# atsuki-ichikawa/KoeMorph

Measured on AMD Instinct MI355X. Metric: blendshape frames/sec (52-coef, 256-win, d_model=256), higher is better.
Workload: dtype f32; 1 GPU; C2: 256 windows/GPU x 136448 samples (8.5 s @16 kHz) -> 1024-pt STFT, hop 533, 80-bin log-mel (257 frames) -> dual-stream attention d_model=256, 8 heads, window 256 -> 52 coefficients + EMA; from audio resident in HBM (rotating batches); windows_per_gpu=256, samples_per_window=136448, parallelism=window-sharded x1, no collective

## Files before the change

koemorph_amd/csrc/km_context.h:

```cpp
#pragma once

#include <cstdint>
#include <map>
#include <string>
#include <vector>

#include "koemorph.h"
#include "km_devbuf.h"

namespace km {

constexpr int kNumMouth = 28;
constexpr int kNumExpr = 24;
extern const int kMouthIdx[kNumMouth];
extern const int kExprIdx[kNumExpr];

struct HostParam {
    std::vector<int64_t> shape;
    std::vector<float> data;
    bool loaded = false;
};

struct Packed {
    std::vector<float> host;
// ... 2 lines not shown

constexpr int kMelRpWaves = 8;
constexpr int kMelRpGroups = 4;
constexpr int kMelRpRow = 580;

struct MelPlan {
    km_mel_config cfg{};
    int n_freq = 0;
    std::vector<float> window;
    std::vector<float> twiddle;
    std::vector<int32_t> fb_start;
    std::vector<int32_t> fb_count;
    std::vector<int32_t> fb_offset;
    std::vector<float> fb_weight;
    std::vector<int32_t> fbg_gid;
    std::vector<int32_t> fbg_desc;
    std::vector<float> fbg_weight;
    int fbg_extent = 0;
    DevBuf<float> d_window, d_twiddle;
    DevBuf<int32_t> d_fb_start, d_fb_count, d_fb_offset;
    DevBuf<float> d_fb_weight;
    DevBuf<int32_t> d_fbg_gid, d_fbg_desc;
    DevBuf<float> d_fbg_weight;
    bool uploaded = false;
};

struct Options {
    int core_split = 0;
    int seq_per_window = 0;
    int seq_assemble = 0;
    int generic_staged = 0;
    int mel_two_frame = 0;
    int emotion_separate = 0;
    int no_ln_fusion = 0, no_db_fusion = 0, no_score_fusion = 0, no_out_fusion = 0, no_v_fusion = 0;
    int legacy_no_merge = 0;
    int no_core_merge = 0;
    int core128 = 0;
    int legacy_no_tail_fusion = 0;
    int legacy_no_enc_fusion = 0;
    int legacy_no_attn_fusion = 0;
    int kmm_no_fuse = 0;
    int train_no_split = 0;
    int train_split_min_k = 0;
    int train_alone_max = 0;
    int train_no_dy_split = 0;
    int train_ln_fuse_rows = 0;
    int train_no_ln_fuse = 0;
    int train_colsum_gemm = 0;
    int train_no_fe_pack = 0;
    int train_attn_regs = 0;
    int train_no_dma = 0;
    int train_op_per_launch = 0;
    int train_bm32_below = 0;
    int train_tail_groups = 0;
};
void options_from_env(Options& o);
int set_option(struct Context* c, const char* name, long long value);

struct PerDeviceOnce {
    unsigned long long seen[4] = {0, 0, 0, 0};
    bool first(int device) {
        if (device < 0 || device >= 256) return true;
        const unsigned long long bit = 1ull << (device & 63);
        if (seen[device >> 6] & bit) return false;
        seen[device >> 6] |= bit;
        return true;
// ... 299 lines not shown
```

koemorph_amd/csrc/km_device.h:

```cpp
#pragma once

#include <hip/hip_runtime.h>

#include "koemorph.h"

namespace km {

struct LogParams {
    int log_mode;
    float amin, top_db, db_add, db_scale, log_eps;
};

__device__ __forceinline__ float clamp_lo(float x, float lo) { return __builtin_amdgcn_fmed3f(x, lo, __builtin_inff()); }
__device__ __forceinline__ float db10(float s, float amin) {
    return 3.01029995663981195f * __builtin_amdgcn_logf(clamp_lo(s, amin));
}

__device__ __forceinline__ void log_window_consts(const LogParams& p, float ref, float& ref_db, float& floor_db) {
    ref_db = db10(ref, p.amin);
    floor_db = (db10(ref, p.amin) - ref_db) - p.top_db;
}

__device__ __forceinline__ float db_finish(const LogParams& p, float dbs, float ref_db, float floor_db) {
    float v = dbs - ref_db;
// ... 32 lines not shown
__device__ __forceinline__ float log_one_t(const LogParams& p, float s, float ref_db, float floor_db) {
    if (MODE == KM_LOG_LN_EPS) return 0.693147180559945309f * __builtin_amdgcn_logf(s + p.log_eps);
    float v = db10(s, p.amin) - ref_db;
    v = clamp_lo(v, floor_db);
    return (v + p.db_add) * p.db_scale;
}

__device__ __forceinline__ float log_one(const LogParams& p, float s, float ref_db, float floor_db) {
    return p.log_mode == KM_LOG_LN_EPS ? log_one_t<KM_LOG_LN_EPS>(p, s, ref_db, floor_db)
                                       : log_one_t<KM_LOG_DB_MAX>(p, s, ref_db, floor_db);
}

template <int MODE>
__device__ __forceinline__ float4 log_four_t(const LogParams& p, float4 v, float ref_db, float floor_db) {
    return make_float4(log_one_t<MODE>(p, v.x, ref_db, floor_db), log_one_t<MODE>(p, v.y, ref_db, floor_db),
                       log_one_t<MODE>(p, v.z, ref_db, floor_db), log_one_t<MODE>(p, v.w, ref_db, floor_db));
}

__device__ __forceinline__ float row16_sum(float v) {
    v += __int_as_float(__builtin_amdgcn_update_dpp(0, __float_as_int(v), 0xB1, 0xF, 0xF, true));
    v += __int_as_float(__builtin_amdgcn_update_dpp(0, __float_as_int(v), 0x4E, 0xF, 0xF, true));
    v += __int_as_float(__builtin_amdgcn_update_dpp(0, __float_as_int(v), 0x141, 0xF, 0xF, true));
    v += __int_as_float(__builtin_amdgcn_update_dpp(0, __float_as_int(v), 0x140, 0xF, 0xF, true));
    return v;
}

struct EmoArgs {
    const float* emo = nullptr;
    int ED = 0;
    const float *wee_t = nullptr , *bee = nullptr, *lg = nullptr, *lb = nullptr, *we2 = nullptr, *be2 = nullptr,
                *w2 = nullptr, *b2 = nullptr;
    float* zemo = nullptr;
    int d = 256, DH = 128;
};

__device__ __forceinline__ void emotion_window_d256(const EmoArgs& e, int64_t b, float* scratch) {
    constexpr int d = 256, DH = 128;
    float* emo_s = scratch;
    float* e1 = scratch + 256;
    float* part = scratch + 512;
    const int tid = threadIdx.x, lane = tid & 63;
    if (tid < 256) emo_s[tid] = tid < e.ED ? e.emo[b * e.ED + tid] : 0.f;
    __syncthreads();
    {
        const int n = tid & 255, h = __builtin_amdgcn_readfirstlane(tid >> 8);
#pragma unroll 1
        for (int q = 2 * h; q < 2 * h + 2; ++q) {
            const float* wp = e.wee_t + (size_t)64 * q * d + n;
            float w[64];
#pragma unroll
            for (int u = 0; u < 64; ++u) w[u] = wp[u * d];
            float acc = 0.f;
#pragma unroll
            for (int u = 0; u < 64; u += 4) {
                const float4 x = *reinterpret_cast<const float4*>(emo_s + 64 * q + u);
                acc = fmaf(x.x, w[u], acc);
                acc = fmaf(x.y, w[u + 1], acc);
                acc = fmaf(x.z, w[u + 2], acc);
                acc = fmaf(x.w, w[u + 3], acc);
            }
            part[q * d + n] = acc;
        }
    }
    __syncthreads();
    if (tid < 256) {
        float s = e.bee[tid];
#pragma unroll
        for (int q = 0; q < 4; ++q) s += part[q * d + tid];
        e1[tid] = s;
    }
    __syncthreads();
    if (tid < 64) {
        float x[4], s = 0.f;
#pragma unroll
        for (int i = 0; i < 4; ++i) { x[i] = e1[lane + 64 * i]; s += x[i]; }
#pragma unroll
        for (int o = 32; o > 0; o >>= 1) s += __shfl_xor(s, o);
        const float mean = s * (1.0f / d);
        float v = 0.f;
#pragma unroll
        for (int i = 0; i < 4; ++i) { const float t = x[i] - mean; v += t * t; }
#pragma unroll
        for (int o = 32; o > 0; o >>= 1) v += __shfl_xor(v, o);
        const float rstd = 1.0f / sqrtf(v * (1.0f / d) + 1e-5f);
#pragma unroll
        for (int i = 0; i < 4; ++i) {
            const int c = lane + 64 * i;
            e1[c] = (x[i] - mean) * rstd * e.lg[c] + e.lb[c];
        }
    }
    __syncthreads();
    {
        const int m = tid & 127, h = tid >> 7;
#pragma unroll 1
        for (int q = 2 * h; q < 2 * h + 2; ++q) {
            const float* wp = e.we2 + (size_t)32 * q * DH + m;
            float w[32];
#pragma unroll
            for (int u = 0; u < 32; ++u) w[u] = wp[u * DH];
            float acc = 0.f;
#pragma unroll
            for (int u = 0; u < 32; u += 4) {
                const float4 x = *reinterpret_cast<const float4*>(e1 + 32 * q + u);
                acc = fmaf(x.x, w[u], acc);
                acc = fmaf(x.y, w[u + 1], acc);
                acc = fmaf(x.z, w[u + 2], acc);
                acc = fmaf(x.w, w[u + 3], acc);
            }
            part[q * DH + m] = acc;
        }
    }
    __syncthreads();
    if (tid < 64) {
        float s = 0.f;
#pragma unroll
        for (int i = 0; i < 2; ++i) {
            const int mm = lane + 64 * i;
            float hsum = e.be2[mm];
#pragma unroll
            for (int q = 0; q < 8; ++q) hsum += part[q * DH + mm];
            s += fmaxf(hsum, 0.f) * e.w2[mm];
        }
#pragma unroll
        for (int o = 32; o > 0; o >>= 1) s += __shfl_xor(s, o);
        if (lane == 0) e.zemo[b] = s + e.b2[0];
    }
    __syncthreads();
}

struct EmoShape { int d = 0, DH = 0; };

__device__ __forceinline__ void emotion_layer_f4(const float* __restrict__ w, int K, int N, const float* x, float* part) {
    const int tid = threadIdx.x;
    const int tpr = N >> 2;
    const int G = 512 / tpr;
    const int c4 = tid & (tpr - 1), g = tid / tpr;
    const int kc = (K + G - 1) / G;
    const int k0 = g * kc, k1 = (k0 + kc) < K ? (k0 + kc) : K;
    float4 acc = make_float4(0.f, 0.f, 0.f, 0.f);
    const float* wp = w + 4 * c4;
    for (int k = k0; k < k1; k += 16) {
        float4 wv[16];
#pragma unroll
        for (int u = 0; u < 16; ++u) wv[u] = (k + u) < k1 ? *reinterpret_cast<const float4*>(wp + (size_t)(k + u) * N) : make_float4(0.f, 0.f, 0.f, 0.f);
#pragma unroll
        for (int u = 0; u < 16; ++u) {
            const float xv = (k + u) < k1 ? x[k + u] : 0.f;
            acc.x = fmaf(xv, wv[u].x, acc.x); acc.y = fmaf(xv, wv[u].y, acc.y);
            acc.z = fmaf(xv, wv[u].z, acc.z); acc.w = fmaf(xv, wv[u].w, acc.w);
        }
    }
    *reinterpret_cast<float4*>(part + g * N + 4 * c4) = acc;
}

__device__ __forceinline__ void emotion_window_generic(const EmoArgs& e, const EmoShape sh, int64_t b, float* scratch) {
    const int d = sh.d, DH = sh.DH;
    float* emo_s = scratch;
    float* e1 = scratch + 256;
    float* part = e1 + d;
    const int tid = threadIdx.x, lane = tid & 63;
    if (tid < 256) emo_s[tid] = tid < e.ED ? e.emo[b * e.ED + tid] : 0.f;
// ... 45 lines not shown
```

koemorph_amd/csrc/km_host.cpp:

```cpp
#include <cctype>
#include <cmath>
#include <cstdlib>
#include <cstdarg>
#include <cstdio>
#include <cstring>

#include "km_context.h"
#include "km_kmmf.h"

namespace km {

const int kMouthIdx[kNumMouth] = {14, 15, 16, 17, 18, 19, 20, 21, 22, 23, 24, 25, 26, 27,
                                  28, 29, 30, 31, 32, 33, 34, 35, 36, 37, 38, 39, 40, 51};
const int kExprIdx[kNumExpr] = {0, 1, 2, 3, 4, 5, 6, 7, 8, 9, 10, 11, 12, 13,
                                41, 42, 43, 44, 45, 46, 47, 48, 49, 50};

static thread_local char g_err[512] = "";

void set_error(const char* fmt, ...) {
    va_list ap;
    va_start(ap, fmt);
    vsnprintf(g_err, sizeof(g_err), fmt, ap);
    va_end(ap);
}
// ... 576 lines not shown
                            (int32_t)((uint32_t)(st4 / 4) | ((uint32_t)steps << 8) | ((uint32_t)(off / 4) << 16));
                        p->fbg_extent = std::max(p->fbg_extent, st4 + 4 * steps);
                    }
                }
            if (p->fbg_extent > kMelRpRow || p->fbg_weight.size() / 4 > 65535) { p->fbg_gid.clear(); p->fbg_desc.clear(); }
        }
        if (p->fbg_weight.empty()) p->fbg_weight.assign(4, 0.0f);
    }
    return p;
}

static bool same_cfg(const km_mel_config& a, const km_mel_config& b) { return std::memcmp(&a, &b, sizeof(a)) == 0; }

MelPlan* find_or_add_plan(Context* c, const km_mel_config& cfg) {
    for (MelPlan* p : c->mel_plans)
        if (same_cfg(p->cfg, cfg)) return p;
    MelPlan* p = build_mel_plan(cfg);
    c->mel_plans.push_back(p);
    return p;
}

}

using namespace km;

namespace km { const char* last_error(); }

namespace km {
namespace {
struct OptName { const char* name; int Options::*field; };
const OptName kOptNames[] = {
    {"core_split", &Options::core_split}, {"seq_per_window", &Options::seq_per_window}, {"seq_assemble", &Options::seq_assemble},
    {"generic_staged", &Options::generic_staged}, {"mel_two_frame", &Options::mel_two_frame},
    {"emotion_separate", &Options::emotion_separate}, {"no_ln_fusion", &Options::no_ln_fusion},
    {"no_db_fusion", &Options::no_db_fusion}, {"no_score_fusion", &Options::no_score_fusion},
    {"no_out_fusion", &Options::no_out_fusion}, {"no_v_fusion", &Options::no_v_fusion}, {"no_core_merge", &Options::no_core_merge}, {"core128", &Options::core128}, {"legacy_no_merge", &Options::legacy_no_merge}, {"kmm_no_fuse", &Options::kmm_no_fuse}, {"legacy_no_attn_fusion", &Options::legacy_no_attn_fusion}, {"legacy_no_enc_fusion", &Options::legacy_no_enc_fusion}, {"legacy_no_tail_fusion", &Options::legacy_no_tail_fusion},
    {"train_no_split", &Options::train_no_split}, {"train_tail_groups", &Options::train_tail_groups}, {"train_bm32_below", &Options::train_bm32_below}, {"train_op_per_launch", &Options::train_op_per_launch}, {"train_split_min_k", &Options::train_split_min_k}, {"train_no_dma", &Options::train_no_dma}, {"train_attn_regs", &Options::train_attn_regs}, {"train_no_fe_pack", &Options::train_no_fe_pack}, {"train_colsum_gemm", &Options::train_colsum_gemm}, {"train_no_ln_fuse", &Options::train_no_ln_fuse}, {"train_ln_fuse_rows", &Options::train_ln_fuse_rows}, {"train_no_dy_split", &Options::train_no_dy_split}, {"train_alone_max", &Options::train_alone_max},
};
}

void options_from_env(Options& o) {
    for (const OptName& n : kOptNames) {
        std::string env = "KM_";
        for (const char* p = n.name; *p; ++p) env += (char)std::toupper((unsigned char)*p);
        if (const char* v = std::getenv(env.c_str())) o.*(n.field) = *v ? std::atoi(v) : 1;
    }
    if (std::getenv("KM_GENERIC_NO_LN_FUSION")) o.no_ln_fusion = 1;
    if (std::getenv("KM_GENERIC_NO_DB_FUSION")) o.no_db_fusion = 1;
    if (std::getenv("KM_GENERIC_NO_SCORE_FUSION")) o.no_score_fusion = 1;
    if (std::getenv("KM_GENERIC_NO_OUT_FUSION")) o.no_out_fusion = 1;
    if (std::getenv("KM_GENERIC_NO_V_FUSION")) o.no_v_fusion = 1;
}

int set_option(Context* c, const char* name, long long value) {
    for (const OptName& n : kOptNames)
        if (std::strcmp(n.name, name) == 0) {
            c->opt.*(n.field) = (int)value;
            return KM_OK;
        }
    return fail(KM_ERR_INVALID_ARG, "km_set_option: unknown option '%s'", name);
}
}

extern "C" {

int km_abi_version(void) { return KM_ABI_VERSION; }
const char* km_last_error(void) { return km::last_error(); }
// ... 273 lines not shown
```

koemorph_amd/csrc/km_mel.hip:

```cpp
#include <hip/hip_runtime.h>

#include <cstdlib>

#include "km_context.h"
#include "km_device.h"

namespace km {


namespace mel {
constexpr int FPB = 16;
constexpr int WAVES = 4;
constexpr int FFT_BUF = 1152;
}

__device__ __forceinline__ float2 cadd(float2 a, float2 b) { return make_float2(a.x + b.x, a.y + b.y); }
__device__ __forceinline__ float2 csub(float2 a, float2 b) { return make_float2(a.x - b.x, a.y - b.y); }
__device__ __forceinline__ float2 cmul(float2 a, float2 b) {
    return make_float2(a.x * b.x - a.y * b.y, a.x * b.y + a.y * b.x);
}

template <int R>
__device__ __forceinline__ float2 twiddle_const(float2 d, int idx) {
    const int s = idx * (16 / R);
// ... 255 lines not shown
                const int st = fbs[m], cnt = fbc[m];
                const float* wt = fbw + fbo[m];
                const float* pr = pw + fl * NFS + st;
                float acc = 0.f;
                if (fvalid) {
#pragma unroll 4
                    for (int i = par; i < cnt; i += 2) acc = fmaf(pr[i], wt[i], acc);
                }
                acc += __shfl_xor(acc, 16);
                if (par == 0) outs[fl * a.n_mels + m] = acc;
                vmax = fmaxf(vmax, acc);
            }
        }
        __syncthreads();
        const int nf_here = (a.n_frames - f0) < FPB ? (a.n_frames - f0) : FPB;
        float* dst = a.melpow + ((int64_t)b * a.n_frames + f0) * a.n_mels;
        for (int i = tid; i < nf_here * a.n_mels; i += 256) dst[i] = outs[i];
    }
#pragma unroll
    for (int o = 32; o > 0; o >>= 1) vmax = fmaxf(vmax, __shfl_xor(vmax, o));
    if (lane == 0) redmax[wave] = vmax;
    __syncthreads();
    if (tid == 0) {
        const float mx = fmaxf(fmaxf(redmax[0], redmax[1]), fmaxf(redmax[2], redmax[3]));
        atomicMax(a.melmax + b, __float_as_uint(mx));
    }
}

#ifndef KM_MEL_SKIP
#define KM_MEL_SKIP 0
#endif
#ifdef KM_MEL_STAMP
#define KM_ASM asm volatile
__device__ unsigned long long km_mel_stamps[1024 * 8 * 24];
#define KM_STAMP(i)                                                  \
    do {                                                             \
        const unsigned long long now_ = __builtin_readcyclecounter(); \
        st_acc[i] += (unsigned)(now_ - st_last);                     \
        st_last = now_;                                              \
    } while (0)
#else
#define KM_ASM asm
#define KM_STAMP(i) do {} while (0)
#endif
namespace melrp {
constexpr int WAVES = kMelRpWaves, NT = 64 * WAVES, FPB = 16, NC = 512, FFT_BUF = 576, NGW = kMelRpGroups;
constexpr int NFS = kMelRpRow;
static_assert(WAVES == 8 && NFS % 64 == 4 && NFS >= 528, "mel stage layout");

typedef float v2f __attribute__((ext_vector_type(2)));

#define KM_ADD(D, A, B) "v_pk_add_f32 %[" #D "], %[" #A "], %[" #B "]\n\t"
#define KM_SUB(D, A, B) "v_pk_add_f32 %[" #D "], %[" #A "], %[" #B "] neg_lo:[0,1] neg_hi:[0,1]\n\t"
#define KM_ADD_NI(D, A, B) "v_pk_add_f32 %[" #D "], %[" #A "], %[" #B "] op_sel:[0,1] op_sel_hi:[1,0] neg_hi:[0,1]\n\t"
#define KM_SUB_NI(D, A, B) "v_pk_add_f32 %[" #D "], %[" #A "], %[" #B "] op_sel:[0,1] op_sel_hi:[1,0] neg_lo:[0,1]\n\t"
#define KM_ROT3(D, S) "v_pk_add_f32 %[" #D "], %[" #S "], %[" #S "] op_sel:[1,0] op_sel_hi:[0,1] neg_lo:[0,1] neg_hi:[1,1]\n\t"
#define KM_CMUL1(T, A, W) "v_pk_mul_f32 %[" #T "], %[" #A "], %[" #W "] op_sel_hi:[0,1]\n\t"
#define KM_CMUL2(D, A, W, T) \
    "v_pk_fma_f32 %[" #D "], %[" #A "], %[" #W "], %[" #T "] op_sel:[1,1,0] op_sel_hi:[1,0,1] neg_lo:[1,0,0]\n\t"

__device__ __forceinline__ void dif8(v2f (&v)[8]) {
    constexpr float C2 = 0.70710678118654752f;
    const v2f c = {C2, C2};
    v2f r0 = v[0], r1 = v[1], r2 = v[2], r3 = v[3], r4 = v[4], r5 = v[5], r6 = v[6], r7 = v[7], t;
    KM_ASM("s_nop 0\n\t"
        KM_ADD(t, r0, r4) KM_SUB(r4, r0, r4)
        KM_ADD(r0, r1, r5) KM_SUB(r5, r1, r5)
// ... 68 lines not shown
                 "ds_read_b64 %5, %8 offset:%14\n\t"
                 "ds_read_b64 %6, %8 offset:%15\n\t"
                 "ds_read_b64 %7, %8 offset:%16\n\t"
                 "s_waitcnt lgkmcnt(0)"
                 : "=&v"(y[0]), "=&v"(y[1]), "=&v"(y[2]), "=&v"(y[3]), "=&v"(y[4]), "=&v"(y[5]), "=&v"(y[6]), "=&v"(y[7])
                 : "v"(addr), "i"(0 * S), "i"(1 * S), "i"(2 * S), "i"(3 * S), "i"(4 * S), "i"(5 * S), "i"(6 * S), "i"(7 * S)
                 : "memory");
}
template <int S>
__device__ __forceinline__ void lds_write8_bitrev(unsigned addr, const v2f (&y)[8]) {
    asm volatile("ds_write_b64 %8, %0 offset:%9\n\t"
                 "ds_write_b64 %8, %1 offset:%10\n\t"
                 "ds_write_b64 %8, %2 offset:%11\n\t"
                 "ds_write_b64 %8, %3 offset:%12\n\t"
                 "ds_write_b64 %8, %4 offset:%13\n\t"
                 "ds_write_b64 %8, %5 offset:%14\n\t"
                 "ds_write_b64 %8, %6 offset:%15\n\t"
                 "ds_write_b64 %8, %7 offset:%16"
                 :
                 : "v"(y[0]), "v"(y[1]), "v"(y[2]), "v"(y[3]), "v"(y[4]), "v"(y[5]), "v"(y[6]), "v"(y[7]), "v"(addr),
                   "i"(0 * S), "i"(4 * S), "i"(2 * S), "i"(6 * S), "i"(1 * S), "i"(5 * S), "i"(3 * S), "i"(7 * S)
                 : "memory");
}
__device__ __forceinline__ v2f ld2(const float2* p) { const float2 t = *p; return v2f{t.x, t.y}; }

#ifndef KM_MEL_XCHG
#define KM_MEL_XCHG 1
#endif
#ifndef KM_MEL_REMAP
#define KM_MEL_REMAP 1
#endif
#ifndef KM_MEL_FLAT
#define KM_MEL_FLAT 0
#endif
#ifndef KM_MEL_PRIO
#define KM_MEL_PRIO 3
#endif
#ifndef KM_MEL_W2
#define KM_MEL_W2 0
#endif
__device__ __forceinline__ void swap_lane32(v2f& a, v2f& b) {
    const auto r0 = __builtin_amdgcn_permlane32_swap(__float_as_uint(a.x), __float_as_uint(b.x), false, false);
    const auto r1 = __builtin_amdgcn_permlane32_swap(__float_as_uint(a.y), __float_as_uint(b.y), false, false);
    a = v2f{__uint_as_float(r0[0]), __uint_as_float(r1[0])}; b = v2f{__uint_as_float(r0[1]), __uint_as_float(r1[1])};
}
__device__ __forceinline__ void swap_lane16(v2f& a, v2f& b) {
    const auto r0 = __builtin_amdgcn_permlane16_swap(__float_as_uint(a.x), __float_as_uint(b.x), false, false);
    const auto r1 = __builtin_amdgcn_permlane16_swap(__float_as_uint(a.y), __float_as_uint(b.y), false, false);
    a = v2f{__uint_as_float(r0[0]), __uint_as_float(r1[0])}; b = v2f{__uint_as_float(r0[1]), __uint_as_float(r1[1])};
}
#define KM_XM " row_mask:0xf bank_mask:"
#define KM_XBANK(CT, MT, CA, MA, MB)                                      \
    "s_nop 1\n\t"                                                        \
    "v_mov_b32_dpp %[t0], %[a0] " CT KM_XM MT "\n\t"                      \
    "v_mov_b32_dpp %[t1], %[a1] " CT KM_XM MT "\n\t"                      \
    "v_mov_b32_dpp %[t2], %[a2] " CT KM_XM MT "\n\t"                      \
    "v_mov_b32_dpp %[t3], %[a3] " CT KM_XM MT "\n\t"                      \
    "v_mov_b32_dpp %[a0], %[b0] " CA KM_XM MA "\n\t"                      \
    "v_mov_b32_dpp %[a1], %[b1] " CA KM_XM MA "\n\t"                      \
    "v_mov_b32_dpp %[a2], %[b2] " CA KM_XM MA "\n\t"                      \
    "v_mov_b32_dpp %[a3], %[b3] " CA KM_XM MA "\n\t"                      \
    "v_mov_b32_dpp %[b0], %[t0] quad_perm:[0,1,2,3]" KM_XM MB "\n\t"      \
    "v_mov_b32_dpp %[b1], %[t1] quad_perm:[0,1,2,3]" KM_XM MB "\n\t"      \
    "v_mov_b32_dpp %[b2], %[t2] quad_perm:[0,1,2,3]" KM_XM MB "\n\t"      \
    "v_mov_b32_dpp %[b3], %[t3] quad_perm:[0,1,2,3]" KM_XM MB "\n\t"      \
    "s_nop 0"
// ... 164 lines not shown
    const int bx = TAB ? (b == 0 ? (int)blockIdx.x : 0) : (int)(lin_ / gridDim.y);
#else
    const int b = blockIdx.y, bx = (int)blockIdx.x;
    static_assert(!TAB, "the clip-span launch is laid out for KM_MEL_REMAP");
#endif
    const unsigned gx = TAB ? (b == 0 ? (unsigned)a.tab_span_wgs : 1u) : gridDim.x;
    const int n_frames = TAB && b > 0 ? 2 : a.n_frames;
    const int64_t gw = a.win0 + b;
    const int64_t clip = TAB ? 0 : gw / a.wins_per_clip;
    int tab_f0 = 0;
    if constexpr (TAB) { tab_f0 = b == 0 ? a.tab_min : a.tab_start[b - 1]; tab_f0 = tab_f0 < 0 ? 0 : tab_f0; }
    const int64_t woff = TAB ? (int64_t)tab_f0 * a.hop : (gw - clip * a.wins_per_clip) * a.win_step;
    const int64_t Lw = TAB ? (int64_t)(b == 0 ? a.n_frames - 1 : a.tab_T) * a.hop : a.L;
    const float* x = a.audio + clip * a.clip_len + (TAB && woff >= a.clip_len ? 0 : woff);
    const int Lv = (int)((a.clip_len - woff) < Lw ? (a.clip_len - woff) : Lw);
    if (a.ready && !a.ready[b]) return;
    const int rs = RING ? a.ring_start[b] : -1;
    v2f* buf = reinterpret_cast<v2f*>(fbuf + wave * FFT_BUF);
    const int n_chunks = (n_frames + FPB - 1) / FPB;
    const unsigned rd2 = lds_offset(buf + (lane >> 3) * 72 + (lane & 7)), rd3 = lds_offset(buf + lane * 9);
    const unsigned wr3 = lds_offset(buf + fft_lane_k0(lane) * 9 + (lane & 7));
    const int cbin = fft_lane_bin(lane);

    v2f zn[8];
    bool zn_ok = false;
    const int fmul = TAB ? (b == 0 ? 1 : a.tab_T) : a.frame_mul;
    auto first_frame = [&]() {
        if (KM_MEL_SKIP & 8) {
#pragma unroll
            for (int i = 0; i < 8; ++i) zn[i] = v2f{0.001f * lane, 0.5f + i};
            zn_ok = true;
        } else if (bx * FPB + wave < n_frames) zn_ok = load_frame_rp_fast<RING>(x, Lv, rs, a.hop, (bx * FPB + wave) * fmul, lane, zn);
    };
    if (!PACK && !TAB && !(KM_MEL_SKIP & 16) && a.emo.emo && bx == (int)gx - 1) {
        if (a.emo.d == 256 && a.emo.DH == 128) emotion_window_d256(a.emo, gw, pw);
        else emotion_window_generic(a.emo, EmoShape{a.emo.d, a.emo.DH}, gw, pw);
        first_frame();
    } else {
        first_frame();
    }

    const unsigned ctr_last = (unsigned)n_chunks - 1u;
    for (int i = tid; i < a.fbg_nw; i += NT) fbw[i] = a.fbg_weight[i];
    for (int i = tid; i < FPB * (NFS - 513); i += NT) pw[(i / (NFS - 513)) * NFS + 513 + i % (NFS - 513)] = 0.f;

    const int n2 = lane & 7, k0 = fft_lane_k0(lane);
    v2f win2[8], tw1[8], tw2[8], twp[4];
#pragma unroll
    for (int i = 0; i < 8; ++i) {
        win2[i] = v2f{a.window[2 * (lane + 64 * i)], a.window[2 * (lane + 64 * i) + 1]};
        tw1[i] = ld2(a.twiddle + ((2 * lane * bitrev(i, 3)) & 1023));
        tw2[i] = ld2(a.twiddle + ((16 * n2 * bitrev(i, 3)) & 1023));
    }
#pragma unroll
    for (int i = 0; i < 4; ++i) twp[i] = ld2(a.twiddle + cbin + 64 * i);

    int my_gid[NGW];
#pragma unroll
    for (int i = 0; i < NGW; ++i) my_gid[i] = __builtin_amdgcn_readfirstlane(a.fbg_gid[wave * NGW + i]);
    const int* my_desc_p = a.fbg_desc + wave * NGW * 4 + mel_slot_of_lane(lane);
#pragma unroll
    for (int i = 0; i < 8; ++i) asm volatile("" ::"v"(win2[i]), "v"(tw1[i]), "v"(tw2[i]));
#pragma unroll
    for (int i = 0; i < 4; ++i) asm volatile("" ::"v"(twp[i]));
#pragma unroll
    for (int i = 0; i < NGW; ++i) asm volatile("" ::"s"(my_gid[i]));

    float vmax = 0.f;
// ... 184 lines not shown
                    acc = __builtin_elementwise_fma(v2f{pv.z, pv.w}, v2f{wv.z, wv.w}, acc);
                    pv = pn; wv = wn;
                }
                acc = __builtin_elementwise_fma(v2f{pv.x, pv.y}, v2f{wv.x, wv.y}, acc);
                acc = __builtin_elementwise_fma(v2f{pv.z, pv.w}, v2f{wv.z, wv.w}, acc);
                float r = acc.x + acc.y;
                r = fvalid ? r : 0.f;
                asm("v_max_f32 %0, %0, %1" : "+v"(vmax) : "v"(r));
                asm("v_max_f32 %0, %0, %1" : "+v"(fmx) : "v"(r));
                store_mel(my_gid[i], r);
            }
#endif
            if (!TAB && a.frame_max) {
                float fall = fmx;
#pragma unroll
                for (int s2 = 0; s2 < 4; ++s2) fall = fmaxf(fall, __shfl(fmx, mel_lane_of(s2, flm)));
                fmx = fall;
                if (slot == 0 && fvalid) atomicMax(a.frame_max + (int64_t)b * n_frames + f0 + flm, __float_as_uint(fmx));
            }
        }
        if (KM_MEL_PRIO) __builtin_amdgcn_s_setprio(0);
        KM_STAMP(10);
        chunk = chunk_next;
        chunk_next = __builtin_amdgcn_readfirstlane(sched[0]);
        __syncthreads();
        KM_STAMP(11);
#ifdef KM_MEL_STAMP
        if (f0 + FPB > n_frames) st_acc[14] += (unsigned)(st_last - st_turn);
        else { st_acc[15] += (unsigned)(st_last - st_turn); }
#endif
    }
#ifdef KM_MEL_STAMP
    if (lane == 0) {
        unsigned long long* o = km_mel_stamps + ((size_t)(b * gridDim.x + bx) * WAVES + wave) * 24;
        if (b * gridDim.x + bx < 1024) {
            for (int i = 0; i < 12; ++i) o[i] = st_acc[i];
            o[12] = st_last - st_first;
            o[13] = st_entry; o[14] = st_first; o[15] = st_last; o[16] = st_entry_rt; o[17] = __builtin_amdgcn_s_memrealtime();
            o[18] = __builtin_readcyclecounter();
            o[19] = st_acc[12]; o[20] = st_acc[13]; o[21] = st_acc[14]; o[22] = st_acc[15];
        }
    }
#endif
#pragma unroll
    for (int o = 32; o > 0; o >>= 1) vmax = fmaxf(vmax, __shfl_xor(vmax, o));
    if (lane == 0) redmax[wave] = vmax;
    __syncthreads();
    if (!TAB && tid == 0 && !a.frame_max) {
        float mx = redmax[0];
#pragma unroll
        for (int w = 1; w < WAVES; ++w) mx = fmaxf(mx, redmax[w]);
        atomicMax(a.melmax + b, __float_as_uint(mx));
    }
}

struct LogArgs {
    const float* melpow;
    const unsigned* melmax;
    int n_frames, out_frames, n_mels;
    LogParams lp;
    float* mel_long;
    float* mel_short;
};

__global__ __launch_bounds__(256) void mel_log_kernel(LogArgs a) {
    const int b = blockIdx.y;
    float ref_db, floor_db;
    log_window_consts(a.lp, __uint_as_float(a.melmax[b]), ref_db, floor_db);
    const float* src = a.melpow + (int64_t)b * a.n_frames * a.n_mels;
    const int total = a.out_frames * a.n_mels;
    const int i = blockIdx.x * 256 + threadIdx.x;
    if (i < total) {
        int f = i / a.n_mels;
// ... 63 lines not shown
                    3 * n_mels + nnz) * sizeof(float);
}

static LogParams log_params(const km_mel_config& m) {
    LogParams lp;
    lp.log_mode = m.log_mode; lp.amin = m.amin; lp.top_db = m.top_db; lp.db_add = m.db_add;
    lp.db_scale = m.db_scale; lp.log_eps = m.log_eps;
    return lp;
}

int growth_refused(void* stream, const char* what, int64_t need, int64_t cap) {
    hipStreamCaptureStatus cs = hipStreamCaptureStatusNone;
    if (hipStreamIsCapturing((hipStream_t)stream, &cs) == hipSuccess && cs != hipStreamCaptureStatusNone)
        return fail(KM_ERR_WORKSPACE, "%s: %lld exceeds the %lld allocated during a stream capture: run one call with this span first",
                    what, (long long)need, (long long)cap);
    return KM_OK;
}

int ensure_chunk_counters(Context* c, int64_t windows, void* stream) {
    if (windows <= c->ws_chunkctr.n) return KM_OK;
    const int64_t cap_n = windows < 4096 ? 4096 : windows;
    if (int rc = c->ws_chunkctr.grow(cap_n, stream, "front end: windows of one launch")) return rc;
    HIP_TRY(hipMemsetAsync(c->ws_chunkctr, 0, (size_t)cap_n * sizeof(unsigned), (hipStream_t)stream));
    HIP_TRY(hipStreamSynchronize((hipStream_t)stream));
    return KM_OK;
}

bool mel_rp_ok(Context* c, MelPlan* p) { return p->cfg.n_fft == 1024 && !c->opt.mel_two_frame && p->d_fbg_gid != nullptr; }

bool clip_frames_shared(Context* c, MelPlan* p) {
    const km_mel_config& m = p->cfg;
    return m.pad_mode == KM_PAD_CONSTANT && 2 * m.hop_length >= m.n_fft && m.n_mels == c->NK && c->NK % 4 == 0;
}

bool mel_fuses_emotion(Context* c, MelPlan* p) {
    auto pow2 = [](int v) { return v >= 64 && v <= 1024 && (v & (v - 1)) == 0; };
    static const bool generic_ok = std::getenv("KM_EMOTION_GENERIC_SEPARATE") == nullptr;
    const bool d256 = c->d == 256 && c->DH == 128;
    return mel_rp_ok(c, p) && !c->opt.emotion_separate && c->kind == 0 && c->ED <= 256 && (d256 || (generic_ok && pow2(c->d) && pow2(c->DH)));
}

bool mel_packs(Context* c, MelPlan* p, int64_t n_frames, int64_t T) {
    const km_mel_config& m = p->cfg;
    return mel_rp_ok(c, p) && m.log_mode == KM_LOG_DB_MAX && m.top_db == m.db_add && m.db_scale > 0.f && n_frames >= T && n_frames >= 3;
}

static void mel_plan_args(MelPlan* p, MelArgs& a) {
    const km_mel_config& m = p->cfg;
    a.hop = m.hop_length; a.pad_mode = m.pad_mode;
    a.n_mels = m.n_mels; a.window = p->d_window; a.twiddle = reinterpret_cast<const float2*>(p->d_twiddle.p);
    a.fb_start = p->d_fb_start; a.fb_count = p->d_fb_count; a.fb_offset = p->d_fb_offset; a.fb_weight = p->d_fb_weight;
    a.fb_nnz = (int)p->fb_weight.size();
    a.fbg_gid = p->d_fbg_gid; a.fbg_desc = p->d_fbg_desc; a.fbg_weight = p->d_fbg_weight; a.fbg_nw = (int)p->fbg_weight.size();
}

int launch_mel_power(Context* c, MelPlan* p, const MelSrc& src, void* stream, const MelCarry& carry) {
    const km_mel_config& m = p->cfg;
    const SeqFrames* seq = carry.seq;
    const int64_t B = src.B, L = src.L;
    const int64_t n_frames = seq ? seq->n_rows : 1 + L / m.hop_length;
    if (m.pad_mode == KM_PAD_REFLECT && L <= m.n_fft / 2)
        return fail(KM_ERR_INVALID_ARG, "reflect padding needs more than n_fft/2 = %d samples (got %lld)", m.n_fft / 2, (long long)L);
    if (!seq && (B > c->ws.windows || n_frames > c->ws.frames))
        return fail(KM_ERR_WORKSPACE, "workspace holds %lld windows x %lld frames, need %lld x %lld: call km_reserve",
                    (long long)c->ws.windows, (long long)c->ws.frames, (long long)B, (long long)n_frames);
    if (!seq && m.n_mels > c->ws.mels)
// ... 6 lines not shown
    if (!p->uploaded) return fail(KM_ERR_NOT_FINALIZED, "mel plan not uploaded (km_finalize / km_reserve first)");
    static PerDeviceOnce once;
    if (once.first(c->device)) {
        const struct { const void* fn; int lds; } kernels[] = {
            {(const void*)&mel_power_kernel<1024, false>, (int)mel_lds_bytes(1024)}, {(const void*)&mel_power_kernel<512, false>, (int)mel_lds_bytes(512)},
            {(const void*)&mel_power_kernel<1024, true>, (int)mel_lds_bytes(1024)}, {(const void*)&mel_power_kernel<512, true>, (int)mel_lds_bytes(512)},
            {(const void*)&mel_power_rp_kernel<false>, 160 * 1024}, {(const void*)&mel_power_rp_kernel<true>, 160 * 1024},
            {(const void*)&mel_power_rp_kernel<false, true>, 160 * 1024}};
        for (const auto& k : kernels) HIP_TRY(hipFuncSetAttribute(k.fn, hipFuncAttributeMaxDynamicSharedMemorySize, k.lds));
    }
    hipStream_t st = (hipStream_t)stream;
    if (int rc = ensure_chunk_counters(c, B, stream)) return rc;
    if (!seq && c->melmax_dirty) {
        HIP_TRY(hipMemsetAsync(c->ws.melmax, 0, (size_t)c->ws.windows * sizeof(unsigned), st));
        c->melmax_dirty = false;
    }
    MelArgs a;
    mel_plan_args(p, a);
    a.audio = src.audio; a.L = L; a.clip_len = src.clip_len; a.win_step = src.win_step; a.win0 = src.win0;
    a.wins_per_clip = src.wins_per_clip > 0 ? src.wins_per_clip : 1; a.n_frames = (int)n_frames;
    a.ring_start = src.ring_start; a.ready = src.ready;
    a.melpow = c->ws.melpow; a.melmax = c->ws.melmax;
    a.frame_mul = 1; a.frame_max = nullptr; a.chunk_ctr = c->ws_chunkctr;
    a.pack_xt = nullptr; a.pack_T = a.pack_KP = 0; a.pack_amin = m.amin;
    a.tab_start = nullptr; a.tab_edge = nullptr; a.tab_min = a.tab_T = a.tab_span_wgs = 0;
    if (carry.pack) { a.pack_xt = carry.pack->xt; a.pack_T = carry.pack->T; a.pack_KP = carry.pack->KP; }
    if (seq) { a.melpow = seq->pow; a.frame_max = seq->fmax; a.frame_mul = seq->frame_mul; a.melmax = nullptr; }
    if (carry.emotion) {
        auto dvp = [&](const char* name) { return (const float*)c->packed.at(name).dev; };
        a.emo.emo = carry.emotion; a.emo.ED = c->ED; a.emo.zemo = carry.zemo;
        a.emo.d = c->d; a.emo.DH = c->DH;
        a.emo.wee_t = (c->d == 256 && c->DH == 128) ? dvp("wee_t256") : dvp("wee_t"); a.emo.bee = dvp("bee"); a.emo.lg = dvp("eln_g"); a.emo.lb = dvp("eln_b");
        a.emo.we2 = dvp("we2"); a.emo.be2 = dvp("be2"); a.emo.w2 = dvp("w2"); a.emo.b2 = dvp("b2");
    }
    const int n_chunks = (int)((n_frames + mel::FPB - 1) / mel::FPB);
    int per_window = (int)((512 + B / 2) / B);
    if (per_window > n_chunks) per_window = n_chunks;
    if (per_window < 1) per_window = 1;
    const dim3 grid((unsigned)per_window, (unsigned)B);
    if (mel_rp_ok(c, p)) {
        const size_t ldsrp = melrp_lds_bytes(a.fbg_nw);
        if (carry.pack) hipLaunchKernelGGL((mel_power_rp_kernel<false, true>), grid, dim3(melrp::NT), ldsrp, st, a);
        else if (!ring) hipLaunchKernelGGL((mel_power_rp_kernel<false>), grid, dim3(melrp::NT), ldsrp, st, a);
        else hipLaunchKernelGGL((mel_power_rp_kernel<true>), grid, dim3(melrp::NT), ldsrp, st, a);
        HIP_TRY(hipGetLastError());
        return KM_OK;
    }
    const size_t lds = mel_lds_bytes(m.n_fft, m.n_mels, a.fb_nnz);
    if (m.n_fft == 1024 && !ring) hipLaunchKernelGGL((mel_power_kernel<1024, false>), grid, dim3(256), lds, st, a);
    else if (m.n_fft == 1024) hipLaunchKernelGGL((mel_power_kernel<1024, true>), grid, dim3(256), lds, st, a);
    else if (!ring) hipLaunchKernelGGL((mel_power_kernel<512, false>), grid, dim3(256), lds, st, a);
    else hipLaunchKernelGGL((mel_power_kernel<512, true>), grid, dim3(256), lds, st, a);
    HIP_TRY(hipGetLastError());
    return KM_OK;
}

struct ClipPackArgs {
    const float* span;
    int edge_off;
    const int* start;
    int min_start, n_span, T, KP, n_mels, row_stride, tile_cols;
    float amin;
    float* xt;
    unsigned* melmax;
};
namespace clippack {
// ... 151 lines not shown
                                 unsigned char* __restrict__ ready, const float* __restrict__ samples,
                                 int n_in, int hop, int ring_len) {
    const int s = blockIdx.x;
    const int w0 = wptr[s];
    float* r = ring + (int64_t)s * ring_len;
    const float* in = samples + (int64_t)s * n_in;
    for (int i = threadIdx.x; i < hop; i += blockDim.x) {
        int p = w0 + i;
        p -= p >= ring_len ? ring_len : 0;
        r[p] = i < n_in ? in[i] : 0.f;
    }
    __syncthreads();
    if (threadIdx.x == 0) {
        int w = w0 + hop;
        w -= w >= ring_len ? ring_len : 0;
        wptr[s] = w;
        const int f = frames[s] + 1;
        frames[s] = f;
        if ((int64_t)f * hop >= ring_len) ready[s] = 1;
    }
}

int launch_ring_push(Context* c, const float* samples, int64_t n_per_stream, void* stream) {
    hipLaunchKernelGGL(ring_push_kernel, dim3((unsigned)c->st.n_streams), dim3(256), 0, (hipStream_t)stream, c->st.ring,
                       c->st.ring_wptr, c->st.ring_frames, c->st.ring_ready, samples, (int)n_per_stream, c->st.ring_hop,
                       (int)c->st.ring_len);
    HIP_TRY(hipGetLastError());
    return KM_OK;
}

LogParams plan_log_params(MelPlan* p) { return log_params(p->cfg); }

#ifdef KM_MEL_STAMP
extern "C" __attribute__((visibility("default"))) int km_debug_mel_stamps(unsigned long long* out, int n) {
    return (int)hipMemcpyFromSymbol(out, HIP_SYMBOL(km_mel_stamps), (size_t)n * sizeof(unsigned long long));
}
#endif

}
```

Baseline: 1.926 million frames/s.

## Batch emotion MLP across groups of windows in a single rider block

The emotion MLP, which rides on the last mel block of each window, now processes 2 (default) or 4 windows per rider block. Each weight column loaded into registers is reused across several windows' inputs. One window per group becomes the rider and the others skip emotion work. This cuts weight traffic and the number of blocks doing the extra work, but makes the rider blocks longer, which could worsen load imbalance. Debug cycle-stamp slots are also added under a compile flag.

```diff
diff --git a/koemorph_amd/csrc/km_context.h b/koemorph_amd/csrc/km_context.h
--- a/koemorph_amd/csrc/km_context.h
+++ b/koemorph_amd/csrc/km_context.h
@@ -58,6 +58,7 @@
     int generic_staged = 0;
     int mel_two_frame = 0;
     int emotion_separate = 0;
+    int emo_group = 0;
     int no_ln_fusion = 0, no_db_fusion = 0, no_score_fusion = 0, no_out_fusion = 0, no_v_fusion = 0;
     int legacy_no_merge = 0;
     int no_core_merge = 0;
diff --git a/koemorph_amd/csrc/km_device.h b/koemorph_amd/csrc/km_device.h
--- a/koemorph_amd/csrc/km_device.h
+++ b/koemorph_amd/csrc/km_device.h
@@ -88,16 +88,20 @@
                 *w2 = nullptr, *b2 = nullptr;
     float* zemo = nullptr;
     int d = 256, DH = 128;
+    int group = 1;
 };
 
-__device__ __forceinline__ void emotion_window_d256(const EmoArgs& e, int64_t b, float* scratch) {
+#define KM_EMO_STAMP(i) do { if (st) st[i] = __builtin_readcyclecounter(); } while (0)
+__device__ __forceinline__ void emotion_window_d256(const EmoArgs& e, int64_t b, float* scratch, unsigned long long* st = nullptr) {
     constexpr int d = 256, DH = 128;
     float* emo_s = scratch;
     float* e1 = scratch + 256;
     float* part = scratch + 512;
     const int tid = threadIdx.x, lane = tid & 63;
+    KM_EMO_STAMP(0);
     if (tid < 256) emo_s[tid] = tid < e.ED ? e.emo[b * e.ED + tid] : 0.f;
     __syncthreads();
+    KM_EMO_STAMP(1);
     {
         const int n = tid & 255, h = __builtin_amdgcn_readfirstlane(tid >> 8);
 #pragma unroll 1
@@ -118,6 +122,7 @@
             part[q * d + n] = acc;
         }
     }
+    KM_EMO_STAMP(2);
     __syncthreads();
     if (tid < 256) {
         float s = e.bee[tid];
@@ -146,6 +151,7 @@
         }
     }
     __syncthreads();
+    KM_EMO_STAMP(3);
     {
         const int m = tid & 127, h = tid >> 7;
 #pragma unroll 1
@@ -166,6 +172,7 @@
             part[q * DH + m] = acc;
         }
     }
+    KM_EMO_STAMP(4);
     __syncthreads();
     if (tid < 64) {
         float s = 0.f;
@@ -182,7 +189,135 @@
         if (lane == 0) e.zemo[b] = s + e.b2[0];
     }
     __syncthreads();
-}
+    KM_EMO_STAMP(5);
+}
+
+constexpr int kEmoGroupMax = 4;
+__host__ __device__ constexpr int emotion_group_floats(int nb) { return nb * (256 + 256) + 4 * nb * 256; }
+
+template <int NB>
+__device__ __forceinline__ void emotion_group_d256_n(const EmoArgs& e, int64_t b0, int nb, float* scratch, unsigned long long* st) {
+    constexpr int d = 256, DH = 128;
+    float* emo_s = scratch;
+    float* e1 = scratch + NB * 256;
+    float* part = scratch + NB * 512;
+    const int tid = threadIdx.x, lane = tid & 63, wave = tid >> 6;
+    KM_EMO_STAMP(0);
+    for (int i = tid; i < NB * 256; i += 512) {
+        const int w = i >> 8, k = i & 255;
+        emo_s[i] = (w < nb && k < e.ED) ? e.emo[(b0 + w) * e.ED + k] : 0.f;
+    }
+    __syncthreads();
+    KM_EMO_STAMP(1);
+    {
+        const int n = tid & 255, h = __builtin_amdgcn_readfirstlane(tid >> 8);
+#pragma unroll 1
+        for (int q = 2 * h; q < 2 * h + 2; ++q) {
+            const float* wp = e.wee_t + (size_t)64 * q * d + n;
+            float w[64];
+#pragma unroll
+            for (int u = 0; u < 64; ++u) w[u] = wp[u * d];
+            float acc[NB];
+#pragma unroll
+            for (int v = 0; v < NB; ++v) acc[v] = 0.f;
+#pragma unroll
+            for (int u = 0; u < 64; u += 4)
+#pragma unroll
+                for (int v = 0; v < NB; ++v) {
+                    const float4 x = *reinterpret_cast<const float4*>(emo_s + v * 256 + 64 * q + u);
+                    acc[v] = fmaf(x.x, w[u], acc[v]);
+                    acc[v] = fmaf(x.y, w[u + 1], acc[v]);
+                    acc[v] = fmaf(x.z, w[u + 2], acc[v]);
+                    acc[v] = fmaf(x.w, w[u + 3], acc[v]);
+                    if (v == NB - 1 && u % 16 == 12) __builtin_amdgcn_sched_barrier(0);
+                }
+#pragma unroll
+            for (int v = 0; v < NB; ++v) part[(q * NB + v) * d + n] = acc[v];
+        }
+    }
+    KM_EMO_STAMP(2);
+    __syncthreads();
+    for (int i = tid; i < NB * d; i += 512) {
+        const int v = i >> 8, n = i & 255;
+        float s = e.bee[n];
+#pragma unroll
+        for (int q = 0; q < 4; ++q) s += part[(q * NB + v) * d + n];
+        e1[i] = s;
+    }
+    __syncthreads();
+    if (wave < nb) {
+        float* ew = e1 + wave * d;
+        float x[4], s = 0.f;
+#pragma unroll
+        for (int i = 0; i < 4; ++i) { x[i] = ew[lane + 64 * i]; s += x[i]; }
+#pragma unroll
+        for (int o = 32; o > 0; o >>= 1) s += __shfl_xor(s, o);
+        const float mean = s * (1.0f / d);
+        float v = 0.f;
+#pragma unroll
+        for (int i = 0; i < 4; ++i) { const float t = x[i] - mean; v += t * t; }
+#pragma unroll
+        for (int o = 32; o > 0; o >>= 1) v += __shfl_xor(v, o);
+        const float rstd = 1.0f / sqrtf(v * (1.0f / d) + 1e-5f);
+#pragma unroll
+        for (int i = 0; i < 4; ++i) {
+            const int c = lane + 64 * i;
+            ew[c] = (x[i] - mean) * rstd * e.lg[c] + e.lb[c];
+        }
+    }
+    __syncthreads();
+    KM_EMO_STAMP(3);
+    {
+        const int m = tid & 127, h = tid >> 7;
+#pragma unroll 1
+        for (int q = 2 * h; q < 2 * h + 2; ++q) {
+            const float* wp = e.we2 + (size_t)32 * q * DH + m;
+            float w[32];
+#pragma unroll
+            for (int u = 0; u < 32; ++u) w[u] = wp[u * DH];
+            float acc[NB];
+#pragma unroll
+            for (int v = 0; v < NB; ++v) acc[v] = 0.f;
+#pragma unroll
+            for (int u = 0; u < 32; u += 4)
+#pragma unroll
+                for (int v = 0; v < NB; ++v) {
+                    const float4 x = *reinterpret_cast<const float4*>(e1 + v * d + 32 * q + u);
+                    acc[v] = fmaf(x.x, w[u], acc[v]);
+                    acc[v] = fmaf(x.y, w[u + 1], acc[v]);
+                    acc[v] = fmaf(x.z, w[u + 2], acc[v]);
+                    acc[v] = fmaf(x.w, w[u + 3], acc[v]);
+                    if (v == NB - 1 && u % 16 == 12) __builtin_amdgcn_sched_barrier(0);
+                }
+#pragma unroll
+            for (int v = 0; v < NB; ++v) part[(q * NB + v) * DH + m] = acc[v];
+        }
+    }
+    KM_EMO_STAMP(4);
+    __syncthreads();
+    if (wave < nb) {
+        float s = 0.f;
+#pragma unroll
+        for (int i = 0; i < 2; ++i) {
+            const int mm = lane + 64 * i;
+            float hsum = e.be2[mm];
+#pragma unroll
+            for (int q = 0; q < 8; ++q) hsum += part[(q * NB + wave) * DH + mm];
+            s += fmaxf(hsum, 0.f) * e.w2[mm];
+        }
+#pragma unroll
+        for (int o = 32; o > 0; o >>= 1) s += __shfl_xor(s, o);
+        if (lane == 0) e.zemo[b0 + wave] = s + e.b2[0];
+    }
+    __syncthreads();
+    KM_EMO_STAMP(5);
+}
+
+__device__ __forceinline__ void emotion_group_d256(const EmoArgs& e, int64_t b0, int nb, float* scratch, unsigned long long* st = nullptr) {
+    if (nb <= 2) emotion_group_d256_n<2>(e, b0, nb, scratch, st);
+    else emotion_group_d256_n<kEmoGroupMax>(e, b0, nb, scratch, st);
+}
+#undef KM_EMO_STAMP
 
 struct EmoShape { int d = 0, DH = 0; };
 
diff --git a/koemorph_amd/csrc/km_host.cpp b/koemorph_amd/csrc/km_host.cpp
--- a/koemorph_amd/csrc/km_host.cpp
+++ b/koemorph_amd/csrc/km_host.cpp
@@ -632,7 +632,7 @@
 const OptName kOptNames[] = {
     {"core_split", &Options::core_split}, {"seq_per_window", &Options::seq_per_window}, {"seq_assemble", &Options::seq_assemble},
     {"generic_staged", &Options::generic_staged}, {"mel_two_frame", &Options::mel_two_frame},
-    {"emotion_separate", &Options::emotion_separate}, {"no_ln_fusion", &Options::no_ln_fusion},
+    {"emotion_separate", &Options::emotion_separate}, {"emo_group", &Options::emo_group}, {"no_ln_fusion", &Options::no_ln_fusion},
     {"no_db_fusion", &Options::no_db_fusion}, {"no_score_fusion", &Options::no_score_fusion},
     {"no_out_fusion", &Options::no_out_fusion}, {"no_v_fusion", &Options::no_v_fusion}, {"no_core_merge", &Options::no_core_merge}, {"core128", &Options::core128}, {"legacy_no_merge", &Options::legacy_no_merge}, {"kmm_no_fuse", &Options::kmm_no_fuse}, {"legacy_no_attn_fusion", &Options::legacy_no_attn_fusion}, {"legacy_no_enc_fusion", &Options::legacy_no_enc_fusion}, {"legacy_no_tail_fusion", &Options::legacy_no_tail_fusion},
     {"train_no_split", &Options::train_no_split}, {"train_tail_groups", &Options::train_tail_groups}, {"train_bm32_below", &Options::train_bm32_below}, {"train_op_per_launch", &Options::train_op_per_launch}, {"train_split_min_k", &Options::train_split_min_k}, {"train_no_dma", &Options::train_no_dma}, {"train_attn_regs", &Options::train_attn_regs}, {"train_no_fe_pack", &Options::train_no_fe_pack}, {"train_colsum_gemm", &Options::train_colsum_gemm}, {"train_no_ln_fuse", &Options::train_no_ln_fuse}, {"train_ln_fuse_rows", &Options::train_ln_fuse_rows}, {"train_no_dy_split", &Options::train_no_dy_split}, {"train_alone_max", &Options::train_alone_max},
diff --git a/koemorph_amd/csrc/km_mel.hip b/koemorph_amd/csrc/km_mel.hip
--- a/koemorph_amd/csrc/km_mel.hip
+++ b/koemorph_amd/csrc/km_mel.hip
@@ -311,7 +311,8 @@
 #endif
 #ifdef KM_MEL_STAMP
 #define KM_ASM asm volatile
-__device__ unsigned long long km_mel_stamps[1024 * 8 * 24];
+constexpr int KM_STAMP_SLOTS = 32;
+__device__ unsigned long long km_mel_stamps[1024 * 8 * KM_STAMP_SLOTS];
 #define KM_STAMP(i)                                                  \
     do {                                                             \
         const unsigned long long now_ = __builtin_readcyclecounter(); \
@@ -446,6 +447,9 @@
 #endif
 #ifndef KM_MEL_FLAT
 #define KM_MEL_FLAT 0
+#endif
+#ifndef KM_EMO_LEADER_FIRST
+#define KM_EMO_LEADER_FIRST 1
 #endif
 #ifndef KM_MEL_PRIO
 #define KM_MEL_PRIO 3
@@ -676,8 +680,27 @@
             zn_ok = true;
         } else if (bx * FPB + wave < n_frames) zn_ok = load_frame_rp_fast<RING>(x, Lv, rs, a.hop, (bx * FPB + wave) * fmul, lane, zn);
     };
-    if (!PACK && !TAB && !(KM_MEL_SKIP & 16) && a.emo.emo && bx == (int)gx - 1) {
-        if (a.emo.d == 256 && a.emo.DH == 128) emotion_window_d256(a.emo, gw, pw);
+    bool rider = !PACK && !TAB && !(KM_MEL_SKIP & 16) && a.emo.emo && bx == (int)gx - 1;
+    int grp_b0 = b, grp_nb = 1;
+    if (!PACK && !TAB && !RING && rider && a.emo.group > 1) {
+        static_assert(emotion_group_floats(kEmoGroupMax) <= FPB * NFS, "the group rider's scratch has to fit the power rows it borrows");
+        const int G = a.emo.group, nwin = (int)gridDim.y;
+        const int g = G == 4 ? b >> 2 : b >> 1;
+        grp_b0 = g * G;
+        grp_nb = nwin - grp_b0 < G ? nwin - grp_b0 : G;
+        int lead = KM_EMO_LEADER_FIRST ? 0 : (G == 4 ? (g >> 1) & 3 : (g >> 2) & 1);
+        lead = lead < grp_nb ? lead : grp_nb - 1;
+        rider = b == grp_b0 + lead;
+    }
+#ifdef KM_MEL_STAMP
+    unsigned long long emo_st_[6] = {0, 0, 0, 0, 0, 0};
+    unsigned long long* const emo_st = emo_st_;
+#else
+    unsigned long long* const emo_st = nullptr;
+#endif
+    if (rider) {
+        if (!RING && a.emo.group > 1) emotion_group_d256(a.emo, a.win0 + grp_b0, grp_nb, pw, emo_st);
+        else if (a.emo.d == 256 && a.emo.DH == 128) emotion_window_d256(a.emo, gw, pw, emo_st);
         else emotion_window_generic(a.emo, EmoShape{a.emo.d, a.emo.DH}, gw, pw);
         first_frame();
     } else {
@@ -928,13 +951,15 @@
     }
 #ifdef KM_MEL_STAMP
     if (lane == 0) {
-        unsigned long long* o = km_mel_stamps + ((size_t)(b * gridDim.x + bx) * WAVES + wave) * 24;
+        unsigned long long* o = km_mel_stamps + ((size_t)(b * gridDim.x + bx) * WAVES + wave) * KM_STAMP_SLOTS;
         if (b * gridDim.x + bx < 1024) {
             for (int i = 0; i < 12; ++i) o[i] = st_acc[i];
             o[12] = st_last - st_first;
             o[13] = st_entry; o[14] = st_first; o[15] = st_last; o[16] = st_entry_rt; o[17] = __builtin_amdgcn_s_memrealtime();
             o[18] = __builtin_readcyclecounter();
             o[19] = st_acc[12]; o[20] = st_acc[13]; o[21] = st_acc[14]; o[22] = st_acc[15];
+            o[23] = rider ? (unsigned long long)grp_nb : 0ull;
+            for (int i = 0; i < 6; ++i) o[24 + i] = emo_st_[i];
         }
     }
 #endif
@@ -1064,6 +1089,8 @@
     const km_mel_config& m = p->cfg;
     return m.pad_mode == KM_PAD_CONSTANT && 2 * m.hop_length >= m.n_fft && m.n_mels == c->NK && c->NK % 4 == 0;
 }
+
+constexpr int kEmoGroupDefault = 2;
 
 bool mel_fuses_emotion(Context* c, MelPlan* p) {
     auto pow2 = [](int v) { return v >= 64 && v <= 1024 && (v & (v - 1)) == 0; };
@@ -1136,6 +1163,8 @@
         a.emo.d = c->d; a.emo.DH = c->DH;
         a.emo.wee_t = (c->d == 256 && c->DH == 128) ? dvp("wee_t256") : dvp("wee_t"); a.emo.bee = dvp("bee"); a.emo.lg = dvp("eln_g"); a.emo.lb = dvp("eln_b");
         a.emo.we2 = dvp("we2"); a.emo.be2 = dvp("be2"); a.emo.w2 = dvp("w2"); a.emo.b2 = dvp("b2");
+        const int want = c->opt.emo_group ? c->opt.emo_group : kEmoGroupDefault;
+        a.emo.group = (want == 2 || want == 4) && c->d == 256 && c->DH == 128 && !ring && !src.ready ? want : 1;
     }
     const int n_chunks = (int)((n_frames + mel::FPB - 1) / mel::FPB);
     int per_window = (int)((512 + B / 2) / B);
@@ -1353,6 +1382,7 @@
 LogParams plan_log_params(MelPlan* p) { return log_params(p->cfg); }
 
 #ifdef KM_MEL_STAMP
+extern "C" __attribute__((visibility("default"))) int km_debug_mel_stamp_slots(void) { return KM_STAMP_SLOTS; }
 extern "C" __attribute__((visibility("default"))) int km_debug_mel_stamps(unsigned long long* out, int n) {
     return (int)hipMemcpyFromSymbol(out, HIP_SYMBOL(km_mel_stamps), (size_t)n * sizeof(unsigned long long));
 }
```

After: 1.922 million frames/s. About the same (-0.2%).
